# alipay/PainlessInferenceAcceleration

Hardware: NVIDIA H100
Metric: accepted tokens/sec @ Llama-2-7B 64-draft/8-branch; mean accepted len/step (higher is better)
Workload: dtype bf16

## Files before the change

painlessinferenceacceleration_b200/csrc/gemm_ws.cu:

```cuda
#include <cuda.h>
#include <cuda_bf16.h>
#include <cuda_fp16.h>

#include <new>

#include "common.cuh"

namespace pia {
namespace gemm {

constexpr int BMW = 128;
constexpr int BK = 64;
constexpr int TOK = 64;
constexpr int NTHREADS = 288;
constexpr int PRODUCER_WARP = 8;
constexpr int W_BYTES = BMW * BK * 2, X_BYTES = TOK * BK * 2, STAGE_BYTES = W_BYTES + X_BYTES;
constexpr int XCH_BYTES = TOK * 64 * 2;
constexpr int smem_total(int nstage) { return nstage * STAGE_BYTES + 256 + XCH_BYTES + 1024; }
constexpr int ACC_OFF = 32 * 1024, ACC_LD = TOK + 4;
static_assert(ACC_OFF + BMW * ACC_LD * 4 <= 4 * STAGE_BYTES, "accumulator staging must fit in the pipeline stages");

__device__ __forceinline__ uint32_t smem_u32(const void *p) { return (uint32_t)__cvta_generic_to_shared(p); }
__device__ __forceinline__ void mbar_init(uint32_t bar, int count) {
  asm volatile("mbarrier.init.shared::cta.b64 [%0], %1;" ::"r"(bar), "r"(count));
// ... 179 lines not shown
    for (int t = 0; t < 16; ++t) {
      const float4 a = src[t];
      v[4 * t] = __float_as_uint(a.x); v[4 * t + 1] = __float_as_uint(a.y);
      v[4 * t + 2] = __float_as_uint(a.z); v[4 * t + 3] = __float_as_uint(a.w);
    }
  }
  if (p.cluster) {
    const int cs = p.cluster, RS = BMW / cs;
    cluster_sync_all();
    {
      const int row = q * 32 + lane;
      const int owner = row / RS, rl = row % RS;
      const uint32_t dst = map_to_cta(base + (uint32_t)((split * 16) * RS + rl) * 16, owner);
#pragma unroll
      for (int tq = 0; tq < 16; ++tq)
        st_cluster_f4(dst + (uint32_t)(tq * RS) * 16, __uint_as_float(v[4 * tq]), __uint_as_float(v[4 * tq + 1]),
                      __uint_as_float(v[4 * tq + 2]), __uint_as_float(v[4 * tq + 3]));
    }
    cluster_sync_all();
    {
      const int e = warp * 32 + lane;
      const int rl = e % RS, tg = e / RS;
      const int qpt = RS / 8;
      const int n_out = n0 + split * RS + rl;
      const float4 *buf = reinterpret_cast<const float4 *>(sm);
      __nv_bfloat16 *ob = p.out_bf16 + grp * p.out_group_stride;
      if (n_out < p.N) {
        for (int tq = tg * qpt; tq < (tg + 1) * qpt; ++tq) {
          float4 a = buf[(0 * 16 + tq) * RS + rl];
          for (int src = 1; src < cs; ++src) {
            const float4 b = buf[(src * 16 + tq) * RS + rl];
            a.x += b.x; a.y += b.y; a.z += b.z; a.w += b.w;
          }
          const int t0 = 4 * tq;
          if (t0 < p.rows) ob[(long long)t0 * p.N + n_out] = __float2bfloat16_rn(a.x);
          if (t0 + 1 < p.rows) ob[(long long)(t0 + 1) * p.N + n_out] = __float2bfloat16_rn(a.y);
          if (t0 + 2 < p.rows) ob[(long long)(t0 + 2) * p.N + n_out] = __float2bfloat16_rn(a.z);
          if (t0 + 3 < p.rows) ob[(long long)(t0 + 3) * p.N + n_out] = __float2bfloat16_rn(a.w);
        }
      }
    }
  } else
  if (p.silu) {
    __nv_bfloat16 *xu = reinterpret_cast<__nv_bfloat16 *>(sm + SMEM_BAR + 256);
    __nv_bfloat16 *xg = xu + 32 * 64;
    const int rr = (q & 1) * 32 + lane;
    if (q >= 2) {
#pragma unroll
      for (int t = 0; t < 32; ++t) xu[t * 64 + rr] = __float2bfloat16_rn(__uint_as_float(v[t]));
    } else {
#pragma unroll
      for (int t = 0; t < 32; ++t) xg[t * 64 + rr] = __float2bfloat16_rn(__uint_as_float(v[32 + t]));
    }
    asm volatile("bar.sync 1, 128;" ::: "memory");
    const int col = tile * 64 + rr;
    const int inter = p.N >> 1;
    if (col < inter) {
      const int tb = q < 2 ? 0 : 32;
#pragma unroll
      for (int t = 0; t < 32; ++t) {
        if (tb + t < p.rows) {
          const float g = q < 2 ? __bfloat162float(__float2bfloat16_rn(__uint_as_float(v[t]))) : __bfloat162float(xg[t * 64 + rr]);
          const float u = q < 2 ? __bfloat162float(xu[t * 64 + rr]) : __bfloat162float(__float2bfloat16_rn(__uint_as_float(v[32 + t])));
          const float sg = __bfloat162float(__float2bfloat16_rn(g / (1.f + expf(-g))));
          p.out_bf16[(long long)(tb + t) * inter + col] = __float2bfloat16_rn(sg * u);
        }
      }
    }
  } else
  if (n < p.N) {
    if (p.n_split == 1) {
#pragma unroll
      for (int t = 0; t < TOK; ++t)
        if (t < p.rows) p.out_bf16[grp * p.out_group_stride + (long long)t * p.N + n] = __float2bfloat16_rn(__uint_as_float(v[t]));
    } else {
      float *o = p.out_f32 + (long long)split * TOK * p.N;
#pragma unroll
      for (int t = 0; t < TOK; ++t)
        if (t < p.rows) o[(long long)t * p.N + n] = __uint_as_float(v[t]);
    }
  }
}


struct SkParams {
  int N, n_tiles, n_chunks, rows, max_contrib;
  long long units;
  __nv_bfloat16 *out;
  float *ws;
  int *flags;
};

__host__ __device__ __forceinline__ long long sk_begin(long long b, long long U, int G) { return b * U / G; }
__host__ __device__ __forceinline__ int sk_cta_of(long long x, long long U, int G) {
  int b = (int)(x * G / U);
  while (b + 1 < G && sk_begin(b + 1, U, G) <= x) ++b;
  while (b > 0 && sk_begin(b, U, G) > x) --b;
  return b;
}

constexpr int SK_STAGES = 8;
constexpr int SK_SMEM_BAR = SK_STAGES * STAGE_BYTES;
constexpr int SK_SMEM_TOTAL = SK_SMEM_BAR + 256 + 1024;

__global__ void __launch_bounds__(NTHREADS, 1)
k_gemm_sk(const __grid_constant__ CUtensorMap map_w, const __grid_constant__ CUtensorMap map_x, SkParams p) {
  extern __shared__ uint8_t smem_raw[];
  const uint32_t base = (smem_u32(smem_raw) + 1023u) & ~1023u;
  const int tid = threadIdx.x, warp = tid >> 5, lane = tid & 31;
  const uint32_t bar_full = base + SK_SMEM_BAR, bar_empty = bar_full + 8 * SK_STAGES;
  const int G = gridDim.x, b = blockIdx.x;
  const long long u0 = sk_begin(b, p.units, G), u1 = sk_begin(b + 1, p.units, G);

  if (tid == 0) {
    for (int s = 0; s < SK_STAGES; ++s) { mbar_init(bar_full + 8 * s, 1); mbar_init(bar_empty + 8 * s, 8); }
    asm volatile("fence.mbarrier_init.release.cluster;" ::: "memory");
  }
  __syncwarp();
  pdl_launch_dependents();
  __syncthreads();
  pdl_wait();

  if (warp == PRODUCER_WARP) {
    if (lane == 0) {
      int i = 0;
      for (long long u = u0; u < u1; ++u, ++i) {
        const int tile = (int)(u / p.n_chunks), ch = (int)(u % p.n_chunks);
        const int s = i % SK_STAGES, ph = (i / SK_STAGES) & 1;
        mbar_wait(bar_empty + 8 * s, ph ^ 1);
        mbar_expect_tx(bar_full + 8 * s, STAGE_BYTES);
        const uint32_t wd = base + s * STAGE_BYTES, xd = wd + W_BYTES;
        tma_load_3d(wd, &map_w, bar_full + 8 * s, 0, 0, tile * p.n_chunks + ch);
        tma_load_2d(xd, &map_x, bar_full + 8 * s, ch * BK, 0);
      }
    }
    return;
  }

  const int wg = warp >> 2;
  int i = 0;
  long long u = u0;
  float acc[32];
  while (u < u1) {
    const int tile = (int)(u / p.n_chunks);
    const long long ts = (long long)tile * p.n_chunks;
    long long ue = ts + p.n_chunks;
    if (ue > u1) ue = u1;
    const bool head = (u == ts), whole = head && (ue == ts + p.n_chunks);
#pragma unroll
    for (int j = 0; j < 32; ++j) acc[j] = 0.f;
    for (; u < ue; ++u, ++i) {
      const int s = i % SK_STAGES, ph = (i / SK_STAGES) & 1;
      mbar_wait(bar_full + 8 * s, ph);
      const uint32_t wa = base + s * STAGE_BYTES, xa = wa + W_BYTES;
      mma_stage(acc, wa + wg * 64 * 128, xa);
      __syncwarp();
      if (lane == 0) mbar_arrive(bar_empty + 8 * s);
    }
    if (!head) {
      const int owner = sk_cta_of(ts, p.units, G);
      const int slot = b - owner - 1;
      float *ws = p.ws + ((long long)tile * p.max_contrib + slot) * BMW * TOK;
#pragma unroll
      for (int h = 0; h < 2; ++h) {
        const int r = wg * 64 + frag_row(warp, lane, h);
#pragma unroll
// ... 454 lines not shown
  if (p.cluster) {
    const int cs = p.cluster, RS = BMW / cs;
    cluster_sync_all();
    {
      const int row = q * 32 + lane;
      const int owner = row / RS, rl = row % RS;
      const uint32_t dst = map_to_cta(base + (uint32_t)((split * 16) * RS + rl) * 16, owner);
#pragma unroll
      for (int tq = 0; tq < 16; ++tq) st_cluster_f4(dst + (uint32_t)(tq * RS) * 16, v[4 * tq], v[4 * tq + 1], v[4 * tq + 2], v[4 * tq + 3]);
    }
    cluster_sync_all();
    {
      const int e = warp * 32 + lane;
      const int rl = e % RS, tg = e / RS;
      const int qpt = RS / 8;
      const int n_out = n0 + split * RS + rl;
      const float4 *buf = reinterpret_cast<const float4 *>(sm);
      __nv_bfloat16 *ob = p.out_bf16 + (long long)t0 * p.N;
      for (int tq = tg * qpt; tq < (tg + 1) * qpt; ++tq) {
        float4 a = buf[(0 * 16 + tq) * RS + rl];
        for (int src = 1; src < cs; ++src) {
          const float4 b = buf[(src * 16 + tq) * RS + rl];
          a.x += b.x; a.y += b.y; a.z += b.z; a.w += b.w;
        }
        if (p.bias) { const float bs = p.bias[n_out]; a.x += bs; a.y += bs; a.z += bs; a.w += bs; }
        const int tt = 4 * tq;
        if (tt < rows) ob[(long long)tt * p.N + n_out] = __float2bfloat16_rn(a.x);
        if (tt + 1 < rows) ob[(long long)(tt + 1) * p.N + n_out] = __float2bfloat16_rn(a.y);
        if (tt + 2 < rows) ob[(long long)(tt + 2) * p.N + n_out] = __float2bfloat16_rn(a.z);
        if (tt + 3 < rows) ob[(long long)(tt + 3) * p.N + n_out] = __float2bfloat16_rn(a.w);
      }
    }
  } else if (p.silu) {
    __nv_bfloat16 *xu = reinterpret_cast<__nv_bfloat16 *>(sm + SMEM_BAR + 256);
    __nv_bfloat16 *xg = xu + 32 * 64;
    const int rr = (q & 1) * 32 + lane;
    if (q >= 2) {
#pragma unroll
      for (int t = 0; t < 32; ++t) xu[t * 64 + rr] = __float2bfloat16_rn(v[t]);
    } else {
#pragma unroll
      for (int t = 0; t < 32; ++t) xg[t * 64 + rr] = __float2bfloat16_rn(v[32 + t]);
    }
    asm volatile("bar.sync 1, 128;" ::: "memory");
    const int col = tile * 64 + rr;
    const int inter = p.N >> 1;
    __nv_bfloat16 *ob = p.out_bf16 + (long long)t0 * inter;
    const int tb = q < 2 ? 0 : 32;
#pragma unroll
    for (int t = 0; t < 32; ++t) {
      if (tb + t < rows) {
        const float g = q < 2 ? __bfloat162float(__float2bfloat16_rn(v[t])) : __bfloat162float(xg[t * 64 + rr]);
        const float u = q < 2 ? __bfloat162float(xu[t * 64 + rr]) : __bfloat162float(__float2bfloat16_rn(v[32 + t]));
        const float sg = __bfloat162float(__float2bfloat16_rn(g / (1.f + expf(-g))));
        ob[(long long)(tb + t) * inter + col] = __float2bfloat16_rn(sg * u);
      }
    }
  } else if (p.n_split == 1) {
    if (p.bias) {
      const float bs = p.bias[n];
#pragma unroll
      for (int t = 0; t < TOK; ++t) v[t] += bs;
    }
    __nv_bfloat16 *ob = p.out_bf16 + (long long)t0 * p.N;
#pragma unroll
    for (int t = 0; t < TOK; ++t)
      if (t < rows) ob[(long long)t * p.N + n] = __float2bfloat16_rn(v[t]);
  } else {
    float *o = p.out_f32 + split * p.slice_stride + (long long)t0 * p.N;
#pragma unroll
    for (int t = 0; t < TOK; ++t)
      if (t < rows) o[(long long)t * p.N + n] = v[t];
  }
}

}
}

using namespace pia;
using namespace pia::gemm;

struct pia_gemm_plan {
  CUtensorMap map_w, map_x;
  Params p;
  int nstage;
  int no_pdl;
  int stream_k, sk_grid;
  SkParams sk;
  int fp8, groups, x_rows;
  F8Params f;
  int w4, w4_f16;
  W4Params w;
};

typedef CUresult (*EncodeTiledFn)(CUtensorMap *, CUtensorMapDataType, cuuint32_t, void *, const cuuint64_t *,
                                  const cuuint64_t *, const cuuint32_t *, const cuuint32_t *, CUtensorMapInterleave,
                                  CUtensorMapSwizzle, CUtensorMapL2promotion, CUtensorMapFloatOOBfill);

static EncodeTiledFn get_encode() {
  static EncodeTiledFn fn = nullptr;
  if (!fn) {
    cudaDriverEntryPointQueryResult qres;
    void *ptr = nullptr;
    if (cudaGetDriverEntryPoint("cuTensorMapEncodeTiled", &ptr, cudaEnableDefault, &qres) == cudaSuccess &&
        qres == cudaDriverEntryPointSuccess) fn = (EncodeTiledFn)ptr;
  }
  return fn;
}

static int encode_tiled_w(CUtensorMap *m, const void *base, uint64_t n_blocks) {
  EncodeTiledFn fn = get_encode();
  PIA_REQUIRE(fn, "cuTensorMapEncodeTiled not available in this driver");
  cuuint64_t dims[3] = {(cuuint64_t)BK, (cuuint64_t)BMW, n_blocks};
  cuuint64_t strides[2] = {(cuuint64_t)BK * 2, (cuuint64_t)BK * BMW * 2};
  cuuint32_t box[3] = {BK, BMW, 1};
  cuuint32_t estr[3] = {1, 1, 1};
  CUresult r = fn(m, CU_TENSOR_MAP_DATA_TYPE_BFLOAT16, 3, const_cast<void *>(base), dims, strides, box, estr,
                  CU_TENSOR_MAP_INTERLEAVE_NONE, CU_TENSOR_MAP_SWIZZLE_128B, CU_TENSOR_MAP_L2_PROMOTION_L2_256B,
                  CU_TENSOR_MAP_FLOAT_OOB_FILL_NONE);
  if (r != CUDA_SUCCESS) { set_error("cuTensorMapEncodeTiled failed with CUresult %d", (int)r); return PIA_ERR_CUDA; }
  return PIA_OK;
}

static int encode_2d(CUtensorMap *m, const void *base, uint64_t inner, uint64_t outer, uint32_t box_inner,
                     uint32_t box_outer, CUtensorMapL2promotion promo) {
  static EncodeTiledFn fn = nullptr;
  if (!fn) {
    cudaDriverEntryPointQueryResult qres;
    void *ptr = nullptr;
    PIA_CUDA_CHECK(cudaGetDriverEntryPoint("cuTensorMapEncodeTiled", &ptr, cudaEnableDefault, &qres));
    PIA_REQUIRE(ptr && qres == cudaDriverEntryPointSuccess, "cuTensorMapEncodeTiled not available in this driver");
    fn = (EncodeTiledFn)ptr;
  }
  cuuint64_t dims[2] = {inner, outer};
  cuuint64_t strides[1] = {inner * 2};
  cuuint32_t box[2] = {box_inner, box_outer};
  cuuint32_t estr[2] = {1, 1};
  CUresult r = fn(m, CU_TENSOR_MAP_DATA_TYPE_BFLOAT16, 2, const_cast<void *>(base), dims, strides, box, estr,
                  CU_TENSOR_MAP_INTERLEAVE_NONE, CU_TENSOR_MAP_SWIZZLE_128B, promo, CU_TENSOR_MAP_FLOAT_OOB_FILL_NONE);
  if (r != CUDA_SUCCESS) { set_error("cuTensorMapEncodeTiled failed with CUresult %d", (int)r); return PIA_ERR_CUDA; }
  return PIA_OK;
}

extern "C" int pia_gemm_plan_create(const void *d_w, int N, int K, const void *d_x, int x_rows, int split_k,
                                    int w_tiled, pia_gemm_plan_t **out) {
  PIA_REQUIRE(d_w && d_x && out, "null argument");
  PIA_REQUIRE(N > 0 && K > 0 && K % BK == 0, "K must be a multiple of %d", BK);
  PIA_REQUIRE(x_rows >= TOK, "the activation buffer must hold at least %d rows", TOK);
  PIA_REQUIRE((reinterpret_cast<uintptr_t>(d_w) & 15) == 0 && (reinterpret_cast<uintptr_t>(d_x) & 15) == 0, "operands must be 16-byte aligned");
  pia_gemm_plan *g = new (std::nothrow) pia_gemm_plan();
  PIA_REQUIRE(g, "out of host memory");
  const int n_chunks = K / BK;
  const int want_stream_k = (split_k == -1);
  const int want_cluster = (split_k == -2 || split_k == -4 || split_k == -8) ? -split_k : 0;
  if (split_k < -1 && !want_cluster) { delete g; set_error("cluster split-K supports 2, 4 or 8 CTAs"); return PIA_ERR_INVALID; }
  if (want_cluster) split_k = want_cluster;
  if (split_k < 1) split_k = 1;
  if (split_k > n_chunks) split_k = n_chunks;
  g->p.N = N; g->p.K = K; g->p.n_chunks = n_chunks;
  g->p.chunks_per_split = (n_chunks + split_k - 1) / split_k;
  g->p.n_split = (n_chunks + g->p.chunks_per_split - 1) / g->p.chunks_per_split;
  g->p.rows = TOK; g->p.out_bf16 = nullptr; g->p.out_f32 = nullptr; g->p.silu = 0;
  g->p.groups = 1; g->p.w_group_rows = 0; g->p.x_group_chunks = 0; g->p.out_group_stride = 0;
  g->p.cluster = 0;
  if (want_cluster) {
    if (g->p.n_split != want_cluster) { delete g; set_error("K = %d is too short for %d cluster splits", K, want_cluster); return PIA_ERR_INVALID; }
    g->p.cluster = want_cluster;
  }
  g->p.tiled = w_tiled ? 1 : 0;
  if (w_tiled && N % BMW != 0) { delete g; set_error("a tiled weight needs N %% %d == 0", BMW); return PIA_ERR_INVALID; }
  int rc = w_tiled ? encode_tiled_w(&g->map_w, d_w, (uint64_t)(N / BMW) * n_chunks)
                   : encode_2d(&g->map_w, d_w, (uint64_t)K, (uint64_t)N, BK, BMW, CU_TENSOR_MAP_L2_PROMOTION_L2_256B);
  if (rc == PIA_OK) rc = encode_2d(&g->map_x, d_x, (uint64_t)K, (uint64_t)x_rows, BK, TOK, CU_TENSOR_MAP_L2_PROMOTION_L2_256B);
  if (rc == PIA_OK) {
    int n_sm = 132, dev = 0;
    cudaGetDevice(&dev);
    cudaDeviceGetAttribute(&n_sm, cudaDevAttrMultiProcessorCount, dev);
    const int ctas = ((N + BMW - 1) / BMW) * g->p.n_split;
    g->nstage = ctas <= n_sm ? 8 : 4;
    cudaError_t e = cudaFuncSetAttribute(k_gemm_ws<4>, cudaFuncAttributeMaxDynamicSharedMemorySize, smem_total(4));
    if (e == cudaSuccess) e = cudaFuncSetAttribute(k_gemm_ws<8>, cudaFuncAttributeMaxDynamicSharedMemorySize, smem_total(8));
    if (e != cudaSuccess) { set_error("cudaFuncSetAttribute: %s", cudaGetErrorString(e)); rc = PIA_ERR_CUDA; }
  }
  g->stream_k = 0; g->no_pdl = 0;
  if (rc == PIA_OK && want_stream_k) {
    if (!w_tiled) { delete g; set_error("stream-K needs the tiled weight layout"); return PIA_ERR_INVALID; }
    int n_sm = 132, dev = 0;
    cudaGetDevice(&dev);
    cudaDeviceGetAttribute(&n_sm, cudaDevAttrMultiProcessorCount, dev);
    SkParams &k = g->sk;
    k.N = N; k.n_tiles = N / BMW; k.n_chunks = n_chunks; k.rows = TOK;
    k.units = (long long)k.n_tiles * n_chunks;
    g->sk_grid = (int)(k.units < n_sm ? k.units : n_sm);
    k.max_contrib = 1;
    for (int t = 0; t < k.n_tiles; ++t) {
      const long long ts = (long long)t * n_chunks;
      const int c = sk_cta_of(ts + n_chunks - 1, k.units, g->sk_grid) - sk_cta_of(ts, k.units, g->sk_grid);
      if (c > k.max_contrib) k.max_contrib = c;
    }
    k.out = nullptr;
    cudaError_t e = cudaMalloc((void **)&k.ws, sizeof(float) * (size_t)k.n_tiles * k.max_contrib * BMW * TOK);
    if (e == cudaSuccess) e = cudaMalloc((void **)&k.flags, sizeof(int) * k.n_tiles);
    if (e == cudaSuccess) e = cudaMemset(k.flags, 0, sizeof(int) * k.n_tiles);
    if (e == cudaSuccess) e = cudaFuncSetAttribute(k_gemm_sk, cudaFuncAttributeMaxDynamicSharedMemorySize, SK_SMEM_TOTAL);
    if (e == cudaSuccess) e = cudaDeviceSynchronize();
    if (e != cudaSuccess) { set_error("stream-K plan: %s", cudaGetErrorString(e)); delete g; return PIA_ERR_CUDA; }
    g->stream_k = 1;
    g->p.n_split = 1;
  }
  if (rc != PIA_OK) { delete g; return rc; }
  *out = g;
  return PIA_OK;
}

extern "C" int pia_gemm_plan_destroy(pia_gemm_plan_t *g) {
  if (g) {
    if (g->stream_k) { cudaFree(g->sk.ws); cudaFree(g->sk.flags); }
    delete g;
  }
  return PIA_OK;
}
extern "C" int pia_gemm_plan_set_pdl(pia_gemm_plan_t *g, int on) {
  PIA_REQUIRE(g, "null plan");
  g->no_pdl = on ? 0 : 1;
  return PIA_OK;
}
extern "C" int pia_gemm_plan_splits(const pia_gemm_plan_t *g) {
  if (g && g->fp8) return g->f.cluster ? 1 : g->f.n_split;
  if (g && g->w4) return g->w.cluster ? 1 : g->w.n_split;
  return g ? (g->p.cluster ? 1 : g->p.n_split) : 0;
}
extern "C" int pia_gemm_plan_set_silu(pia_gemm_plan_t *g, int on) {
  if (g && g->fp8) {
    PIA_REQUIRE(g->f.n_split == 1 && !g->f.bias && g->groups == 1,
                "the SiLU*up epilogue needs split_k == 1, no bias and one group");
    PIA_REQUIRE(!on || !g->f.relu, "a plan has one epilogue activation: ReLU is already set");
    g->f.silu = on ? 1 : 0;
    return PIA_OK;
  }
  if (g && g->w4) {
    PIA_REQUIRE(g->w.n_split == 1 && !g->w.bias, "the SiLU*up epilogue needs split_k == 1 and no bias");
    g->w.silu = on ? 1 : 0;
    return PIA_OK;
  }
  PIA_REQUIRE(g && g->p.n_split == 1 && !g->stream_k && g->p.N % BMW == 0, "the SiLU*up epilogue needs split_k == 1 and N %% 128 == 0");
  g->p.silu = on ? 1 : 0;
  return PIA_OK;
}
extern "C" int pia_gemm_plan_set_relu(pia_gemm_plan_t *g, int on) {
  PIA_REQUIRE(g && g->fp8, "the ReLU epilogue exists on fp8 plans only");
  if (on) {
    PIA_REQUIRE(g->f.n_split == 1 || g->f.cluster, "the ReLU epilogue needs bf16 outputs: split_k == 1 or a cluster split");
    PIA_REQUIRE(!g->f.silu, "a plan has one epilogue activation: SiLU*up is already set");
  }
  g->f.relu = on ? 1 : 0;
  return PIA_OK;
}

extern "C" int pia_gemm_plan_create_grouped(const void *d_w, int groups, int N, int K, const void *d_x, int x_rows,
                                            pia_gemm_plan_t **out) {
  PIA_REQUIRE(d_w && d_x && out, "null argument");
  PIA_REQUIRE(groups >= 1 && groups <= 65535 && N > 0 && N % BMW == 0 && K > 0 && K % BK == 0,
              "grouped GEMM needs N %% %d == 0 and K %% %d == 0", BMW, BK);
  PIA_REQUIRE(x_rows >= TOK, "the activation buffer must hold at least %d rows", TOK);
  PIA_REQUIRE((reinterpret_cast<uintptr_t>(d_w) & 15) == 0 && (reinterpret_cast<uintptr_t>(d_x) & 15) == 0, "operands must be 16-byte aligned");
  pia_gemm_plan *g = new (std::nothrow) pia_gemm_plan();
// ... 125 lines not shown
  if (rc == PIA_OK) {
    int n_sm = 132, dev = 0;
    cudaGetDevice(&dev);
    cudaDeviceGetAttribute(&n_sm, cudaDevAttrMultiProcessorCount, dev);
    g->nstage = w.tiles * w.n_split <= n_sm ? 4 : 2;
    cudaError_t e = cudaFuncSetAttribute(k_gemm_w4<2, false>, cudaFuncAttributeMaxDynamicSharedMemorySize, w4_smem_total(2));
    if (e == cudaSuccess) e = cudaFuncSetAttribute(k_gemm_w4<4, false>, cudaFuncAttributeMaxDynamicSharedMemorySize, w4_smem_total(4));
    if (e == cudaSuccess) e = cudaFuncSetAttribute(k_gemm_w4<2, true>, cudaFuncAttributeMaxDynamicSharedMemorySize, w4_smem_total(2));
    if (e == cudaSuccess) e = cudaFuncSetAttribute(k_gemm_w4<4, true>, cudaFuncAttributeMaxDynamicSharedMemorySize, w4_smem_total(4));
    if (e != cudaSuccess) { set_error("cudaFuncSetAttribute: %s", cudaGetErrorString(e)); rc = PIA_ERR_CUDA; }
  }
  if (rc != PIA_OK) { delete g; return rc; }
  *out = g;
  return PIA_OK;
}

extern "C" int pia_gemm_plan_create_w4(const void *d_codes, const void *d_scale, const void *d_zero, int scale_dtype,
                                       const void *d_bias, int N, int K, int group_size, const void *d_x, int x_rows,
                                       int split_k, pia_gemm_plan_t **out) {
  return w4_plan_create(d_codes, d_scale, d_zero, scale_dtype, d_bias, N, K, group_size, d_x, x_rows, split_k, out);
}

struct PdlScope { int on; explicit PdlScope(int off) : on(off) { if (on) ++pia::g_pdl_off; } ~PdlScope() { if (on) --pia::g_pdl_off; } };

static int f8_run(pia_gemm_plan_t *g, int rows, void *d_out, void *stream) {
  PIA_REQUIRE(rows >= 1 && rows <= g->x_rows, "rows %d outside [1,%d]", rows, g->x_rows);
  PdlScope pdl_scope(g->no_pdl);
  F8Params f = g->f;
  f.rows = rows; f.ntb = (rows + TOK - 1) / TOK; f.no_pdl = g->no_pdl;
  if (f.n_split == 1 || f.cluster) f.out_bf16 = (__nv_bfloat16 *)d_out; else f.out_f32 = (float *)d_out;
  const unsigned z = (unsigned)(g->groups * f.ntb);
  const dim3 grid = f.cluster ? dim3(f.n_split, f.tiles, z) : dim3(f.tiles, f.n_split, z);
  const unsigned cs = f.cluster ? (unsigned)f.cluster : 1u;
  if (g->nstage == 6) PIA_CUDA_CHECK(launch_kernel_cluster(k_gemm_fp8<6>, grid, dim3(NTHREADS), f8_smem_total(6), (cudaStream_t)stream, cs, g->map_w, g->map_x, f));
  else PIA_CUDA_CHECK(launch_kernel_cluster(k_gemm_fp8<3>, grid, dim3(NTHREADS), f8_smem_total(3), (cudaStream_t)stream, cs, g->map_w, g->map_x, f));
  count_launch();
  return PIA_OK;
}

static int w4_run(pia_gemm_plan_t *g, int rows, void *d_out, void *stream) {
  PIA_REQUIRE(rows >= 1 && rows <= g->x_rows, "rows %d outside [1,%d]", rows, g->x_rows);
  PdlScope pdl_scope(g->no_pdl);
  W4Params w = g->w;
  w.rows = rows; w.ntb = (rows + TOK - 1) / TOK; w.no_pdl = g->no_pdl;
  if (w.n_split == 1 || w.cluster) w.out_bf16 = (__nv_bfloat16 *)d_out; else w.out_f32 = (float *)d_out;
  const dim3 grid = w.cluster ? dim3(w.n_split, w.tiles, w.ntb) : dim3(w.tiles, w.n_split, w.ntb);
  const unsigned cs = w.cluster ? (unsigned)w.cluster : 1u;
  const cudaStream_t st = (cudaStream_t)stream;
  if (g->nstage == 4) {
    if (g->w4_f16) PIA_CUDA_CHECK(launch_kernel_cluster(k_gemm_w4<4, true>, grid, dim3(NTHREADS), w4_smem_total(4), st, cs, g->map_w, g->map_x, w));
    else PIA_CUDA_CHECK(launch_kernel_cluster(k_gemm_w4<4, false>, grid, dim3(NTHREADS), w4_smem_total(4), st, cs, g->map_w, g->map_x, w));
  } else {
    if (g->w4_f16) PIA_CUDA_CHECK(launch_kernel_cluster(k_gemm_w4<2, true>, grid, dim3(NTHREADS), w4_smem_total(2), st, cs, g->map_w, g->map_x, w));
    else PIA_CUDA_CHECK(launch_kernel_cluster(k_gemm_w4<2, false>, grid, dim3(NTHREADS), w4_smem_total(2), st, cs, g->map_w, g->map_x, w));
  }
  count_launch();
  return PIA_OK;
}

extern "C" int pia_gemm_run(pia_gemm_plan_t *g, int rows, void *d_out, void *stream) {
  PIA_REQUIRE(g && d_out, "null argument");
  if (g->fp8) return f8_run(g, rows, d_out, stream);
  if (g->w4) return w4_run(g, rows, d_out, stream);
  PIA_REQUIRE(rows >= 1 && rows <= TOK, "rows %d outside [1,%d]", rows, TOK);
  PdlScope pdl_scope(g->no_pdl);
  if (g->stream_k) {
    SkParams k = g->sk;
    k.rows = rows;
    k.out = (__nv_bfloat16 *)d_out;
    PIA_CUDA_CHECK(launch_kernel(k_gemm_sk, dim3(g->sk_grid), dim3(NTHREADS), SK_SMEM_TOTAL, (cudaStream_t)stream, g->map_w, g->map_x, k));
    count_launch();
    return PIA_OK;
  }
  Params p = g->p;
  p.rows = rows; p.no_pdl = g->no_pdl;
  if (p.n_split == 1 || p.cluster) p.out_bf16 = (__nv_bfloat16 *)d_out; else p.out_f32 = (float *)d_out;
  if (p.cluster) {
    dim3 cgrid(p.n_split, (p.N + BMW - 1) / BMW);
    if (g->nstage == 8) PIA_CUDA_CHECK(launch_kernel_cluster(k_gemm_ws<8>, cgrid, dim3(NTHREADS), smem_total(8), (cudaStream_t)stream, (unsigned)p.cluster, g->map_w, g->map_x, p));
    else PIA_CUDA_CHECK(launch_kernel_cluster(k_gemm_ws<4>, cgrid, dim3(NTHREADS), smem_total(4), (cudaStream_t)stream, (unsigned)p.cluster, g->map_w, g->map_x, p));
    count_launch();
    return PIA_OK;
  }
  dim3 grid((p.N + BMW - 1) / BMW, p.n_split, p.groups);
  if (g->nstage == 8) PIA_CUDA_CHECK(launch_kernel(k_gemm_ws<8>, grid, dim3(NTHREADS), smem_total(8), (cudaStream_t)stream, g->map_w, g->map_x, p));
  else PIA_CUDA_CHECK(launch_kernel(k_gemm_ws<4>, grid, dim3(NTHREADS), smem_total(4), (cudaStream_t)stream, g->map_w, g->map_x, p));
  count_launch();
  return PIA_OK;
}
```

painlessinferenceacceleration_b200/models/llama/modeling_llama.py:

```python
import glob
import json
import math
import os

import torch
from torch import nn

from ...common import ops
from ...common.pretrained_model import LookaheadPreTrainedModel


class LlamaRMSNorm(nn.Module):
    def __init__(self, hidden_size, eps=1e-6, device=None, dtype=None):
        super().__init__()
        self.weight = nn.Parameter(torch.ones(hidden_size, device=device, dtype=dtype))
        self.variance_epsilon = eps


class LlamaAttention(nn.Module):
    def __init__(self, cfg, device, dtype, qkv_bias=False):
        super().__init__()
        hd = cfg.hidden_size // cfg.num_attention_heads
        kv = getattr(cfg, 'num_key_value_heads', None) or cfg.num_attention_heads
        kw = dict(bias=False, device=device, dtype=dtype)
# ... 633 lines not shown
        elif rtype == 'dynamic':
            factor, mpe = float(scaling['factor']), int(c.max_position_embeddings)
            if max_pos > mpe:
                base = theta * ((factor * max_pos / mpe) - (factor - 1)) ** (hd / (hd - 2))
                inv_freq = 1.0 / (base ** (torch.arange(0, hd, 2, dtype=torch.int64).float().to(dev) / hd))
        elif rtype == 'llama3':
            factor, low, high = float(scaling['factor']), float(scaling['low_freq_factor']), float(scaling['high_freq_factor'])
            old_ctx = scaling.get('original_max_position_embeddings') or c.max_position_embeddings
            low_freq_wavelen, high_freq_wavelen = old_ctx / low, old_ctx / high
            wavelen = 2 * math.pi / inv_freq
            inv_freq_llama = torch.where(wavelen > low_freq_wavelen, inv_freq / factor, inv_freq)
            smooth_factor = (old_ctx / wavelen - low) / (high - low)
            smoothed_inv_freq = (1 - smooth_factor) * inv_freq_llama / factor + smooth_factor * inv_freq_llama
            is_medium_freq = ~(wavelen < high_freq_wavelen) * ~(wavelen > low_freq_wavelen)
            inv_freq = torch.where(is_medium_freq, smoothed_inv_freq, inv_freq_llama)
        else:
            raise ValueError(f'Unknown RoPE scaling type {rtype}')
        freqs = pos[:, None] * inv_freq[None, :]
        return freqs.cos().to(torch.bfloat16).contiguous(), freqs.sin().to(torch.bfloat16).contiguous()

    def _gemm_plans(self, rt):
        plans = getattr(rt, 'gemm_plans', None)
        if plans is not None:
            return plans
        if self._fp8 or self._w4:
            mk = self._fp8_plans if self._fp8 else self._w4_plans
            mk(rt.decode_bufs)
            mk(rt.prefill_bufs)
            rt.gemm_plans = False
            return False
        import os
        if os.environ.get('PIA_GEMM', '1') == '0' or rt.max_nodes != 64:
            rt.gemm_plans = False
            return False
        b = rt.decode_bufs
        g = rt.g
        dev = b.y.device
        b.gu = torch.zeros((b.rows, 2 * g['inter']), dtype=torch.bfloat16, device=dev)
        b.act = torch.zeros((b.rows, g['inter']), dtype=torch.bfloat16, device=dev)
        plans = {'layers': []}
        for layer in self.model.layers:
            plans['layers'].append(self._layer_gemm_plans(layer, b))
        plans['lm_head'] = self._mk_gemm(self.lm_head.weight.data, b.y)
        rt.gemm_plans = plans
        return plans

    def _layer_gemm_plans(self, layer, b):
        import os
        want = os.environ.get('PIA_GEMM_SET', 'gate_up').split(',')
        if ('qkv' in want or 'qkv2' in want) and layer.self_attn.qkv_bias is not None:
            raise ValueError('PIA_GEMM_SET names qkv, but this model has QKV biases and k_gemm_ws has no bias epilogue')
        plans = {}
        if 'gate_up_silu' in want and layer.mlp.gate_up_weight.shape[0] % 256 == 0:
            cache = self.__dict__.setdefault('_tiled_weights', {})
            key = ('gate_up_silu', layer.mlp.gate_up_weight.data_ptr())
            if key not in cache:
                cache[key] = ops.tile_weight(ops.interleave_gate_up(layer.mlp.gate_up_weight))
            plans['gate_up_silu'] = ops.Gemm(cache[key], b.y, tiled=True).set_silu()
        elif 'gate_up' in want or 'gate_up_silu' in want:
            plans['gate_up'] = self._mk_gemm(layer.mlp.gate_up_weight, b.y)
        if 'qkv' in want:
            plans['qkv'] = self._mk_gemm(layer.self_attn.qkv_weight, b.y)
        sk = int(os.environ.get('PIA_GEMM_SPLIT', '-4'))
        if 'qkv2' in want:
            plans['qkv'] = self._mk_gemm(layer.self_attn.qkv_weight, b.y, split_k=-2)
        if 'o' in want:
            plans['o'] = self._mk_gemm(layer.self_attn.o_proj.weight.data, b.attn, split_k=sk)
        if 'down' in want and layer.mlp.down_proj.weight.shape[1] % 64 == 0 and layer.mlp.down_proj.weight.shape[1] >= 64 * abs(sk):
            plans['down'] = self._mk_gemm(layer.mlp.down_proj.weight.data, b.act, split_k=sk)
        for name in os.environ.get('PIA_GEMM_NOPDL', '').split(','):
            if name in plans:
                plans[name].set_pdl(False)
        return plans

    def _mk_gemm(self, w, x, split_k=1):
        if w.shape[0] % 128 == 0:
            cache = self.__dict__.setdefault('_tiled_weights', {})
            key = (w.data_ptr(), tuple(w.shape))
            if key not in cache:
                cache[key] = ops.tile_weight(w)
            return ops.Gemm(cache[key], x, split_k=split_k, tiled=True)
        return ops.Gemm(w.contiguous(), x, split_k=split_k)

    def _prefetch_cfg(self, rt):
        cfg = getattr(rt, 'prefetch_cfg', None)
        if cfg is None:
            import os
            spec = os.environ.get('PIA_PREFETCH', '0')
            v = [float(t) for t in spec.split(',')] if spec not in ('', '0') else []
            cfg = False
            if v and torch.cuda.is_available():
                v = (v + [0.0] * 4)[:4]
                cfg = dict(o=v[0], gate_up=v[1], down=v[2], rate=v[3], side=torch.cuda.Stream(device=self.device))
            rt.prefetch_cfg = cfg
        return cfg

    @staticmethod
    def _prefetch(pf, jobs):
        main = torch.cuda.current_stream()
        pf['side'].wait_stream(main)
        with torch.cuda.stream(pf['side']):
            for (t, frac, tile_bytes) in jobs:
                if frac <= 0:
                    continue
                total = t.numel() * t.element_size()
                if tile_bytes:
                    rb = max(16384, int(tile_bytes * min(frac, 1.0)) // 16384 * 16384)
                    ops.l2_prefetch(t, n_ranges=total // tile_bytes, stride_bytes=tile_bytes, range_bytes=min(rb, tile_bytes),
                                    gbytes_per_s=pf['rate'])
                else:
                    ops.l2_prefetch(t, range_bytes=int(total * min(frac, 1.0)) // 16 * 16, gbytes_per_s=pf['rate'])
        pf['dirty'] = True

    def _check_fused_attn(self):
        if self.rotary_interleaved and os.environ.get('PIA_ATTN_FUSED', '0') != '0':
            raise ValueError(f'{type(self).__name__} rotates interleaved pairs (GLM RoPE), which the fused attention '
                             'kernel does not: unset PIA_ATTN_FUSED')

    def _mlp(self, rt, layer, y, plans=None, pf=None, b=None):
        m = layer.mlp
        if plans:
            b = b if b is not None else rt.decode_bufs
            rows = y.shape[0]
            if 'gate_up_silu' in plans:
                plans['gate_up_silu'].run(rows, out=b.act)
            else:
                if 'gate_up' in plans:
                    plans['gate_up'].run(64, out=b.gu)
                else:
                    torch.mm(y, m.gate_up_weight.t(), out=b.gu)
                if pf:
                    self._prefetch(pf, [(m.down_proj.weight, pf['down'], 0)])
                ops.silu_mul(b.gu, b.act)
            if 'down' in plans:
                o = plans['down'].run(rows)
                return (o, None) if plans['down'].splits == 1 else (None, o)
            return torch.mm(b.act, m.down_proj.weight.t()), None
        gu = torch.mm(y, m.gate_up_weight.t())
        act = torch.empty((gu.shape[0], gu.shape[1] // 2), dtype=gu.dtype, device=gu.device)
        ops.silu_mul(gu, act)
        return torch.mm(act, m.down_proj.weight.t()), None

    def _verify_layers(self, rt, bufs=None, last_only=False):
        self.fuse()
        b = bufs if bufs is not None else rt.decode_bufs
        g = rt.g
        eps = self.config.rms_norm_eps
        ops.embed_gather(self.model.embed_tokens.weight, b.ids, b.n_total, b.h)
        if self._fp8:
            plans, rows = self._fp8_plans(b), b.rows
        elif self._w4:
            plans, rows = self._w4_plans(b), b.rows
        else:
            plans, rows = (self._gemm_plans(rt) if b is rt.decode_bufs else False), 64
        pf = self._prefetch_cfg(rt) if plans and not (self._fp8 or self._w4) else False
        fused_attn = b is rt.decode_bufs and os.environ.get('PIA_ATTN_FUSED', '0') != '0' and \
            (b.slots.batch == 1 or b.slots.kv_slot_stride != 0)
        if fused_attn:
            self._check_fused_attn()
        rotary_dim = g['rotary_dim'] if self.rotary_interleaved else None
        alibi = getattr(rt, 'alibi_slopes', None)
        logn = getattr(rt, 'logn_scale', None)
        x, parts, resid_in = b.h, None, None

        rnd = self.rmsnorm_rounding

        def norm(w):
            if parts is not None:
                ops.rmsnorm_partials(parts, resid_in, w, eps, b.resid, b.y, rounding=rnd)
            else:
                ops.rmsnorm(x, resid_in, w, eps, b.resid, b.y, rounding=rnd)

        def post_norm(w):
            if parts is not None:
                ops.rmsnorm_partials(parts, None, w, eps, None, b.post_norm, rounding=rnd)
            else:
                ops.rmsnorm(x, None, w, eps, None, b.post_norm, rounding=rnd)
            return b.post_norm, None

        for li, layer in enumerate(self.model.layers):
            lp = plans['layers'][li] if plans else None
            norm(layer.input_layernorm.weight)
            a = layer.self_attn
            if lp and 'qkv' in lp:
                lp['qkv'].run(rows, out=b.qkv)
            elif a.qkv_bias is not None:
                torch.addmm(a.qkv_bias, b.y, a.qkv_weight.t(), out=b.qkv)
            else:
                torch.mm(b.y, a.qkv_weight.t(), out=b.qkv)
            if pf and lp and 'gate_up' in lp:
                gw = lp['gate_up'].weight
                self._prefetch(pf, [(a.o_proj.weight, pf['o'], 0),
                                    (gw, pf['gate_up'], gw.shape[1] * gw.shape[2] * gw.shape[3] * 2 if gw.dim() == 4 else 0)])
            if fused_attn:
                rt.plan.forward_fused(li, b.qkv, b.mask, b.slots, rt.rope_cos, rt.rope_sin, b.attn)
            else:
                ops.rope_kv_append(b.qkv, b.mask, b.slots, g['n_q_heads'], g['n_kv_heads'], g['head_dim'], rt.rope_cos,
                                   rt.rope_sin, b.q, rt.k_layer(li, b.kv_slot), rt.v_layer(li, b.kv_slot), rt.max_seq,
                                   rotary_dim=rotary_dim, q_scale=logn)
                rt.plan.forward(li, b.q, b.mask, b.slots, b.attn, alibi_slopes=alibi)
            if lp and 'o' in lp:
                o = lp['o'].run(rows)
                x, parts, resid_in = (o, None, b.resid) if lp['o'].splits == 1 else (None, o, b.resid)
            else:
                x, parts, resid_in = torch.mm(b.attn, a.o_proj.weight.t()), None, b.resid
            if self.sandwich_norms:
                x, parts = post_norm(layer.post_self_attn_layernorm.weight)
            norm(layer.post_attention_layernorm.weight)
            x, parts = self._mlp(rt, layer, b.y, lp, pf, b=b)
            if self.sandwich_norms:
                x, parts = post_norm(layer.post_mlp_layernorm.weight)
        if pf and pf.pop('dirty', False):
            torch.cuda.current_stream().wait_stream(pf['side'])
        if last_only:
            return
        norm(self.model.norm.weight)
        if b.logits is not None:
            if plans and 'lm_head' in plans:
                plans['lm_head'].run(64, out=b.logits)
            else:
                torch.mm(b.y, self.lm_head.weight.t(), out=b.logits)


class LlamaPreTrainedModel(LookaheadPreTrainedModel):
    pass
```

painlessinferenceacceleration_b200/models/mixtral/modeling_mixtral.py:

```python
import torch
from torch import nn

from ...common import ops
from ..llama.modeling_llama import Fp8Linear, LlamaDecoderLayer, LlamaForCausalLM, LlamaModel
from ..mistral.modeling_mistral import warn_sliding_window


class MixtralRouter(nn.Module):
    def __init__(self, cfg, device, dtype):
        super().__init__()
        self.weight = nn.Parameter(torch.empty((cfg.num_local_experts, cfg.hidden_size), device=device, dtype=dtype))


class MixtralExperts(nn.Module):
    def __init__(self, cfg, device, dtype):
        super().__init__()
        E, H, I = cfg.num_local_experts, cfg.hidden_size, cfg.intermediate_size
        self.gate_up_proj = nn.Parameter(torch.empty((E, 2 * I, H), device=device, dtype=dtype))
        self.down_proj = nn.Parameter(torch.empty((E, H, I), device=device, dtype=dtype))


class MixtralSparseMoeBlock(nn.Module):
    def __init__(self, cfg, device, dtype):
        super().__init__()
# ... 20 lines not shown
    def _fuse_mlp(self, layer):
        pass

    def rope_tables(self, max_pos):
        warn_sliding_window(self.config, max_pos)
        return super().rope_tables(max_pos)

    def _convert_checkpoint_keys(self, sd):
        import re
        out = {}
        pend = self.__dict__.setdefault('_pending_experts', {})
        E = self.config.num_local_experts
        pat = re.compile(r'^(model\.layers\.\d+)\.block_sparse_moe\.experts\.(\d+)\.(w1|w2|w3)\.weight$')
        for k, v in sd.items():
            m = pat.match(k)
            if m:
                pend.setdefault(m.group(1), {})[(int(m.group(2)), m.group(3))] = v
            elif '.block_sparse_moe.gate.weight' in k:
                out[k.replace('.block_sparse_moe.gate.weight', '.mlp.gate.weight')] = v
            else:
                out[k] = v
        for layer in list(pend):
            parts = pend[layer]
            if len(parts) == 3 * E:
                out[layer + '.mlp.experts.gate_up_proj'] = torch.stack(
                    [torch.cat([parts[(e, 'w1')], parts[(e, 'w3')]], dim=0) for e in range(E)], dim=0)
                out[layer + '.mlp.experts.down_proj'] = torch.stack([parts[(e, 'w2')] for e in range(E)], dim=0)
                del pend[layer]
        return out

    def geometry(self):
        g = super().geometry()
        g['n_experts'] = self.config.num_local_experts
        return g

    def _layer_gemm_plans(self, layer, b):
        import os
        moe = layer.mlp
        E, two_i, H = moe.experts.gate_up_proj.shape
        inter = two_i // 2
        if os.environ.get('PIA_MOE_GEMM', '1') == '0' or H % 128 or H % 64 or inter % 64 or (E * two_i) % 128:
            return {}
        dev = b.y.device
        if not hasattr(b, 'moe_gu'):
            b.moe_gu = torch.zeros((b.rows, E * two_i), dtype=torch.bfloat16, device=dev)
            b.moe_act = torch.zeros((b.rows, E * inter), dtype=torch.bfloat16, device=dev)
            b.moe_out = torch.zeros((b.rows, H), dtype=torch.bfloat16, device=dev)
            b.moe_dense = torch.zeros((b.rows, E), dtype=torch.bfloat16, device=dev)
        return {'moe_gate_up': ops.Gemm(moe.experts.gate_up_proj.data.view(E * two_i, H), b.y),
                'moe_down': ops.Gemm.grouped(moe.experts.down_proj.data, b.moe_act)}

    _fp8_params = ('self_attn.q_proj.weight', 'self_attn.k_proj.weight', 'self_attn.v_proj.weight',
                   'self_attn.o_proj.weight', 'mlp.experts.gate_up_proj', 'mlp.experts.down_proj')

    def _fp8_weight_shapes(self, layer):
        a, ex = layer.self_attn, layer.mlp.experts
        return [('qkv', a.qkv_weight.shape), ('o_proj', a.o_proj.weight.shape),
                ('experts.gate_up_proj', ex.gate_up_proj.shape), ('experts.down_proj', ex.down_proj.shape)]

    def _quantize_mlp(self, layer):
        ex = layer.mlp.experts
        gu = Fp8Linear(ex.gate_up_proj.data, interleaved=True)
        del ex.gate_up_proj
        ex.gate_up_proj = gu
        dn = Fp8Linear(ex.down_proj.data)
        del ex.down_proj
        ex.down_proj = dn

    def _layer_fp8_plans(self, layer, b, n_sm):
        plans = self._attn_fp8_plans(layer, b, n_sm)
        ex = layer.mlp.experts
        E, two_i, H = ex.gate_up_proj.shape
        dev = b.y.device
        if getattr(b, 'moe_act', None) is None or b.moe_act.shape[0] != b.rows:
            b.moe_act = torch.zeros((b.rows, E * (two_i // 2)), dtype=torch.bfloat16, device=dev)
            b.moe_out = torch.zeros((b.rows, H), dtype=torch.bfloat16, device=dev)
            b.moe_dense = torch.zeros((b.rows, E), dtype=torch.bfloat16, device=dev)
        gq = ex.gate_up_proj.qweight
        plans['moe_gate_up_silu'] = ops.Gemm.fp8(gq.view(-1, *gq.shape[2:]), ex.gate_up_proj.scale.view(-1), b.y,
                                                 out=b.moe_act).set_silu()
        plans['moe_down'] = ops.Gemm.grouped_fp8(ex.down_proj.qweight, ex.down_proj.scale, b.moe_act)
        return plans

    def _mlp(self, rt, layer, y, plans=None, pf=None, b=None):
        moe = layer.mlp
        if plans:
            b = b if b is not None else rt.decode_bufs
            E = moe.num_experts
            inter = moe.experts.down_proj.shape[2]
            ops.moe_router(y, moe.gate.weight, moe.top_k, b.moe_dense)
            if 'moe_gate_up_silu' in plans:
                rows = y.shape[0]
                plans['moe_gate_up_silu'].run(rows, out=b.moe_act)
                ye = plans['moe_down'].run(rows)
                ops.moe_combine(ye, b.moe_dense, b.moe_out)
                return b.moe_out, None
            plans['moe_gate_up'].run(64, out=b.moe_gu)
            ops.silu_mul(b.moe_gu.view(b.rows * E, 2 * inter), b.moe_act.view(b.rows * E, inter))
            ye = plans['moe_down'].run(64)
            ops.moe_combine(ye, b.moe_dense, b.moe_out)
            return b.moe_out, None
        dense = torch.empty((y.shape[0], moe.num_experts), dtype=y.dtype, device=y.device)
        ops.moe_router(y, moe.gate.weight, moe.top_k, dense)
        out = torch.zeros_like(y)
        inter = moe.experts.down_proj.shape[2]
        act = torch.empty((y.shape[0], inter), dtype=y.dtype, device=y.device)
        for e in range(moe.num_experts):
            gu = torch.mm(y, moe.experts.gate_up_proj[e].t())
            ops.silu_mul(gu, act)
            ye = torch.mm(act, moe.experts.down_proj[e].t())
            w = dense[:, e:e + 1]
            out += torch.where(w != 0, ye * w, 0.0)
        return out, None
```

Before: 575.5.

## Add non-split streaming GEMM kernel with 64-row tiles and drop L2 prefetch path

Adds a new warp-specialized TMA/WGMMA kernel, k_gemm_stream, for the non-split, non-SiLU, single-group case. Each warpgroup owns 64 output rows, and the kernel uses a one-warpgroup variant with 64-row tiles when N is small enough, which launches more CTAs to fill the SMs. Stages are released one WGMMA group late so loads overlap compute. A second 64-row tensor map is encoded for this path. The Python side removes the optional side-stream L2 prefetch code, which was off by default.

```diff
diff --git a/painlessinferenceacceleration_b200/csrc/gemm_ws.cu b/painlessinferenceacceleration_b200/csrc/gemm_ws.cu
--- a/painlessinferenceacceleration_b200/csrc/gemm_ws.cu
+++ b/painlessinferenceacceleration_b200/csrc/gemm_ws.cu
@@ -285,6 +285,101 @@
   }
 }
 
+template <int WG, int NSTAGE>
+__global__ void __launch_bounds__(WG * 128 + 32, WG == 1 ? 3 : (NSTAGE <= 4 ? 2 : 1))
+k_gemm_stream(const __grid_constant__ CUtensorMap map_w, const __grid_constant__ CUtensorMap map_x, Params p) {
+  constexpr int TW_BYTES = WG * 64 * BK * 2, TSTAGE = TW_BYTES + X_BYTES, SMEM_BAR = NSTAGE * TSTAGE;
+  constexpr int NCW = WG * 4;
+  extern __shared__ uint8_t smem_raw[];
+  const uint32_t base = (smem_u32(smem_raw) + 1023u) & ~1023u;
+  uint8_t *sm = smem_raw + (base - smem_u32(smem_raw));
+  const int tid = threadIdx.x, warp = tid >> 5, lane = tid & 31;
+  const uint32_t bar_full = base + SMEM_BAR, bar_empty = bar_full + 8 * NSTAGE;
+  const int tile = blockIdx.x, nch = p.n_chunks;
+  const int n0 = tile * WG * 64;
+
+  if (tid == 0) {
+    for (int s = 0; s < NSTAGE; ++s) { mbar_init(bar_full + 8 * s, 1); mbar_init(bar_empty + 8 * s, NCW); }
+    asm volatile("fence.mbarrier_init.release.cluster;" ::: "memory");
+  }
+  __syncwarp();
+  if (!p.no_pdl) pdl_launch_dependents();
+  __syncthreads();
+
+  if (warp == NCW) {
+    if (lane == 0) {
+      auto load_w = [&](int i, int s) {
+        const uint32_t wd = base + s * TSTAGE;
+        if (p.tiled) tma_load_3d(wd, &map_w, bar_full + 8 * s, 0, 0, WG == 2 ? tile * nch + i : 2 * ((tile >> 1) * nch + i) + (tile & 1));
+        else tma_load_2d(wd, &map_w, bar_full + 8 * s, i * BK, n0);
+      };
+      const int pre = nch < NSTAGE ? nch : NSTAGE;
+      for (int i = 0; i < pre; ++i) {
+        mbar_expect_tx(bar_full + 8 * i, TSTAGE);
+        load_w(i, i);
+      }
+      pdl_wait();
+      for (int i = 0; i < pre; ++i) tma_load_2d(base + i * TSTAGE + TW_BYTES, &map_x, bar_full + 8 * i, i * BK, 0);
+      for (int i = pre; i < nch; ++i) {
+        const int s = i % NSTAGE, ph = (i / NSTAGE) & 1;
+        mbar_wait(bar_empty + 8 * s, ph ^ 1);
+        mbar_expect_tx(bar_full + 8 * s, TSTAGE);
+        load_w(i, s);
+        tma_load_2d(base + s * TSTAGE + TW_BYTES, &map_x, bar_full + 8 * s, i * BK, 0);
+      }
+    }
+    return;
+  }
+
+  pdl_wait();
+  const int wg = warp >> 2;
+  float acc[32];
+#pragma unroll
+  for (int j = 0; j < 32; ++j) acc[j] = 0.f;
+  wgmma_fence();
+  for (int i = 0; i < nch; ++i) {
+    const int s = i % NSTAGE, ph = (i / NSTAGE) & 1;
+    mbar_wait(bar_full + 8 * s, ph);
+    const uint32_t wa = base + s * TSTAGE + wg * 64 * 128, xa = base + s * TSTAGE + TW_BYTES;
+#pragma unroll
+    for (int j = 0; j < BK / 16; ++j) wgmma_m64n64k16(acc, kmajor_desc(wa + j * 32), kmajor_desc(xa + j * 32));
+    wgmma_commit();
+    asm volatile("wgmma.wait_group.sync.aligned 1;" ::: "memory");
+    if (i > 0) {
+      __syncwarp();
+      if (lane == 0) mbar_arrive(bar_empty + 8 * ((i - 1) % NSTAGE));
+    }
+  }
+  wgmma_wait_all();
+  fence_acc(acc);
+
+  float *accs = reinterpret_cast<float *>(sm);
+  asm volatile("bar.sync 2, %0;" ::"n"(NCW * 32) : "memory");
+#pragma unroll
+  for (int h = 0; h < 2; ++h) {
+    const int r = wg * 64 + frag_row(warp, lane, h);
+#pragma unroll
+    for (int i = 0; i < 8; ++i)
+      *reinterpret_cast<float2 *>(accs + r * ACC_LD + frag_tok(lane, i)) = make_float2(acc[4 * i + 2 * h], acc[4 * i + 2 * h + 1]);
+  }
+  asm volatile("bar.sync 2, %0;" ::"n"(NCW * 32) : "memory");
+  const int row = tid % (WG * 64), t0 = (tid / (WG * 64)) * 32;
+  const int n = n0 + row;
+  if (n < p.N) {
+    const float4 *src = reinterpret_cast<const float4 *>(accs + row * ACC_LD + t0);
+#pragma unroll
+    for (int q = 0; q < 8; ++q) {
+      const float4 a = src[q];
+      const int t = t0 + 4 * q;
+      if (t < p.rows) p.out_bf16[(long long)t * p.N + n] = __float2bfloat16_rn(a.x);
+      if (t + 1 < p.rows) p.out_bf16[(long long)(t + 1) * p.N + n] = __float2bfloat16_rn(a.y);
+      if (t + 2 < p.rows) p.out_bf16[(long long)(t + 2) * p.N + n] = __float2bfloat16_rn(a.z);
+      if (t + 3 < p.rows) p.out_bf16[(long long)(t + 3) * p.N + n] = __float2bfloat16_rn(a.w);
+    }
+  }
+}
+template <int WG, int NSTAGE>
+constexpr int stream_smem_total() { return NSTAGE * (WG * 64 * BK * 2 + X_BYTES) + 16 * NSTAGE + 1024; }
 
 struct SkParams {
   int N, n_tiles, n_chunks, rows, max_contrib;
@@ -905,8 +1000,10 @@
 
 struct pia_gemm_plan {
   CUtensorMap map_w, map_x;
+  CUtensorMap map_w64;
   Params p;
   int nstage;
+  int stream_wg;
   int no_pdl;
   int stream_k, sk_grid;
   SkParams sk;
@@ -937,6 +1034,20 @@
   cuuint64_t dims[3] = {(cuuint64_t)BK, (cuuint64_t)BMW, n_blocks};
   cuuint64_t strides[2] = {(cuuint64_t)BK * 2, (cuuint64_t)BK * BMW * 2};
   cuuint32_t box[3] = {BK, BMW, 1};
+  cuuint32_t estr[3] = {1, 1, 1};
+  CUresult r = fn(m, CU_TENSOR_MAP_DATA_TYPE_BFLOAT16, 3, const_cast<void *>(base), dims, strides, box, estr,
+                  CU_TENSOR_MAP_INTERLEAVE_NONE, CU_TENSOR_MAP_SWIZZLE_128B, CU_TENSOR_MAP_L2_PROMOTION_L2_256B,
+                  CU_TENSOR_MAP_FLOAT_OOB_FILL_NONE);
+  if (r != CUDA_SUCCESS) { set_error("cuTensorMapEncodeTiled failed with CUresult %d", (int)r); return PIA_ERR_CUDA; }
+  return PIA_OK;
+}
+
+static int encode_tiled_w64(CUtensorMap *m, const void *base, uint64_t n_blocks) {
+  EncodeTiledFn fn = get_encode();
+  PIA_REQUIRE(fn, "cuTensorMapEncodeTiled not available in this driver");
+  cuuint64_t dims[3] = {(cuuint64_t)BK, 64, 2 * n_blocks};
+  cuuint64_t strides[2] = {(cuuint64_t)BK * 2, (cuuint64_t)BK * 64 * 2};
+  cuuint32_t box[3] = {BK, 64, 1};
   cuuint32_t estr[3] = {1, 1, 1};
   CUresult r = fn(m, CU_TENSOR_MAP_DATA_TYPE_BFLOAT16, 3, const_cast<void *>(base), dims, strides, box, estr,
                   CU_TENSOR_MAP_INTERLEAVE_NONE, CU_TENSOR_MAP_SWIZZLE_128B, CU_TENSOR_MAP_L2_PROMOTION_L2_256B,
@@ -1001,10 +1112,16 @@
     cudaDeviceGetAttribute(&n_sm, cudaDevAttrMultiProcessorCount, dev);
     const int ctas = ((N + BMW - 1) / BMW) * g->p.n_split;
     g->nstage = ctas <= n_sm ? 8 : 4;
+    g->stream_wg = (N + 63) / 64 <= 3 * n_sm ? 1 : 2;
     cudaError_t e = cudaFuncSetAttribute(k_gemm_ws<4>, cudaFuncAttributeMaxDynamicSharedMemorySize, smem_total(4));
     if (e == cudaSuccess) e = cudaFuncSetAttribute(k_gemm_ws<8>, cudaFuncAttributeMaxDynamicSharedMemorySize, smem_total(8));
+    if (e == cudaSuccess) e = cudaFuncSetAttribute(k_gemm_stream<2, 4>, cudaFuncAttributeMaxDynamicSharedMemorySize, stream_smem_total<2, 4>());
+    if (e == cudaSuccess) e = cudaFuncSetAttribute(k_gemm_stream<2, 8>, cudaFuncAttributeMaxDynamicSharedMemorySize, stream_smem_total<2, 8>());
+    if (e == cudaSuccess) e = cudaFuncSetAttribute(k_gemm_stream<1, 4>, cudaFuncAttributeMaxDynamicSharedMemorySize, stream_smem_total<1, 4>());
     if (e != cudaSuccess) { set_error("cudaFuncSetAttribute: %s", cudaGetErrorString(e)); rc = PIA_ERR_CUDA; }
   }
+  if (rc == PIA_OK) rc = w_tiled ? encode_tiled_w64(&g->map_w64, d_w, (uint64_t)(N / BMW) * n_chunks)
+                                 : encode_2d(&g->map_w64, d_w, (uint64_t)K, (uint64_t)N, BK, 64, CU_TENSOR_MAP_L2_PROMOTION_L2_256B);
   g->stream_k = 0; g->no_pdl = 0;
   if (rc == PIA_OK && want_stream_k) {
     if (!w_tiled) { delete g; set_error("stream-K needs the tiled weight layout"); return PIA_ERR_INVALID; }
@@ -1296,6 +1413,17 @@
     count_launch();
     return PIA_OK;
   }
+  if (p.n_split == 1 && !p.silu && p.groups == 1) {
+    const cudaStream_t st = (cudaStream_t)stream;
+    if (g->stream_wg == 1)
+      PIA_CUDA_CHECK(launch_kernel(k_gemm_stream<1, 4>, dim3((p.N + 63) / 64), dim3(160), stream_smem_total<1, 4>(), st, g->map_w64, g->map_x, p));
+    else if (g->nstage == 8)
+      PIA_CUDA_CHECK(launch_kernel(k_gemm_stream<2, 8>, dim3((p.N + BMW - 1) / BMW), dim3(NTHREADS), stream_smem_total<2, 8>(), st, g->map_w, g->map_x, p));
+    else
+      PIA_CUDA_CHECK(launch_kernel(k_gemm_stream<2, 4>, dim3((p.N + BMW - 1) / BMW), dim3(NTHREADS), stream_smem_total<2, 4>(), st, g->map_w, g->map_x, p));
+    count_launch();
+    return PIA_OK;
+  }
   dim3 grid((p.N + BMW - 1) / BMW, p.n_split, p.groups);
   if (g->nstage == 8) PIA_CUDA_CHECK(launch_kernel(k_gemm_ws<8>, grid, dim3(NTHREADS), smem_total(8), (cudaStream_t)stream, g->map_w, g->map_x, p));
   else PIA_CUDA_CHECK(launch_kernel(k_gemm_ws<4>, grid, dim3(NTHREADS), smem_total(4), (cudaStream_t)stream, g->map_w, g->map_x, p));
diff --git a/painlessinferenceacceleration_b200/models/llama/modeling_llama.py b/painlessinferenceacceleration_b200/models/llama/modeling_llama.py
--- a/painlessinferenceacceleration_b200/models/llama/modeling_llama.py
+++ b/painlessinferenceacceleration_b200/models/llama/modeling_llama.py
@@ -739,42 +739,12 @@
             return ops.Gemm(cache[key], x, split_k=split_k, tiled=True)
         return ops.Gemm(w.contiguous(), x, split_k=split_k)
 
-    def _prefetch_cfg(self, rt):
-        cfg = getattr(rt, 'prefetch_cfg', None)
-        if cfg is None:
-            import os
-            spec = os.environ.get('PIA_PREFETCH', '0')
-            v = [float(t) for t in spec.split(',')] if spec not in ('', '0') else []
-            cfg = False
-            if v and torch.cuda.is_available():
-                v = (v + [0.0] * 4)[:4]
-                cfg = dict(o=v[0], gate_up=v[1], down=v[2], rate=v[3], side=torch.cuda.Stream(device=self.device))
-            rt.prefetch_cfg = cfg
-        return cfg
-
-    @staticmethod
-    def _prefetch(pf, jobs):
-        main = torch.cuda.current_stream()
-        pf['side'].wait_stream(main)
-        with torch.cuda.stream(pf['side']):
-            for (t, frac, tile_bytes) in jobs:
-                if frac <= 0:
-                    continue
-                total = t.numel() * t.element_size()
-                if tile_bytes:
-                    rb = max(16384, int(tile_bytes * min(frac, 1.0)) // 16384 * 16384)
-                    ops.l2_prefetch(t, n_ranges=total // tile_bytes, stride_bytes=tile_bytes, range_bytes=min(rb, tile_bytes),
-                                    gbytes_per_s=pf['rate'])
-                else:
-                    ops.l2_prefetch(t, range_bytes=int(total * min(frac, 1.0)) // 16 * 16, gbytes_per_s=pf['rate'])
-        pf['dirty'] = True
-
     def _check_fused_attn(self):
         if self.rotary_interleaved and os.environ.get('PIA_ATTN_FUSED', '0') != '0':
             raise ValueError(f'{type(self).__name__} rotates interleaved pairs (GLM RoPE), which the fused attention '
                              'kernel does not: unset PIA_ATTN_FUSED')
 
-    def _mlp(self, rt, layer, y, plans=None, pf=None, b=None):
+    def _mlp(self, rt, layer, y, plans=None, b=None):
         m = layer.mlp
         if plans:
             b = b if b is not None else rt.decode_bufs
@@ -786,8 +756,6 @@
                     plans['gate_up'].run(64, out=b.gu)
                 else:
                     torch.mm(y, m.gate_up_weight.t(), out=b.gu)
-                if pf:
-                    self._prefetch(pf, [(m.down_proj.weight, pf['down'], 0)])
                 ops.silu_mul(b.gu, b.act)
             if 'down' in plans:
                 o = plans['down'].run(rows)
@@ -810,7 +778,6 @@
             plans, rows = self._w4_plans(b), b.rows
         else:
             plans, rows = (self._gemm_plans(rt) if b is rt.decode_bufs else False), 64
-        pf = self._prefetch_cfg(rt) if plans and not (self._fp8 or self._w4) else False
         fused_attn = b is rt.decode_bufs and os.environ.get('PIA_ATTN_FUSED', '0') != '0' and \
             (b.slots.batch == 1 or b.slots.kv_slot_stride != 0)
         if fused_attn:
@@ -845,10 +812,6 @@
                 torch.addmm(a.qkv_bias, b.y, a.qkv_weight.t(), out=b.qkv)
             else:
                 torch.mm(b.y, a.qkv_weight.t(), out=b.qkv)
-            if pf and lp and 'gate_up' in lp:
-                gw = lp['gate_up'].weight
-                self._prefetch(pf, [(a.o_proj.weight, pf['o'], 0),
-                                    (gw, pf['gate_up'], gw.shape[1] * gw.shape[2] * gw.shape[3] * 2 if gw.dim() == 4 else 0)])
             if fused_attn:
                 rt.plan.forward_fused(li, b.qkv, b.mask, b.slots, rt.rope_cos, rt.rope_sin, b.attn)
             else:
@@ -864,11 +827,9 @@
             if self.sandwich_norms:
                 x, parts = post_norm(layer.post_self_attn_layernorm.weight)
             norm(layer.post_attention_layernorm.weight)
-            x, parts = self._mlp(rt, layer, b.y, lp, pf, b=b)
+            x, parts = self._mlp(rt, layer, b.y, lp, b=b)
             if self.sandwich_norms:
                 x, parts = post_norm(layer.post_mlp_layernorm.weight)
-        if pf and pf.pop('dirty', False):
-            torch.cuda.current_stream().wait_stream(pf['side'])
         if last_only:
             return
         norm(self.model.norm.weight)
diff --git a/painlessinferenceacceleration_b200/models/mixtral/modeling_mixtral.py b/painlessinferenceacceleration_b200/models/mixtral/modeling_mixtral.py
--- a/painlessinferenceacceleration_b200/models/mixtral/modeling_mixtral.py
+++ b/painlessinferenceacceleration_b200/models/mixtral/modeling_mixtral.py
@@ -126,7 +126,7 @@
         plans['moe_down'] = ops.Gemm.grouped_fp8(ex.down_proj.qweight, ex.down_proj.scale, b.moe_act)
         return plans
 
-    def _mlp(self, rt, layer, y, plans=None, pf=None, b=None):
+    def _mlp(self, rt, layer, y, plans=None, b=None):
         moe = layer.mlp
         if plans:
             b = b if b is not None else rt.decode_bufs
```

Result: faster. 596.2, median of 6 (+3.6%).
